# AKGWSB/EzRT

Measured on AMD Instinct MI355X. Metric: Mrays/s at fixed spp (Bunny ~70k tris, 4 bounces), higher is better.
Workload: dtype f32

## Files before the change

### ezrt_amd/csrc/hip/ezrt_device.h

```cpp
#pragma once
#include <hip/hip_runtime.h>
#include <stdint.h>

#include "ezrt.h"
#include "ezrt_detmath.h"

#define EZD __device__ __forceinline__

namespace ezd {

constexpr float PI = EZ_PI;
constexpr float INF = EZ_INF;

struct f3 {
  float x, y, z;
};
EZD f3 mk(float x, float y, float z) { return f3{x, y, z}; }
struct Sample3 {
  float x, y, z;
};
EZD f3 operator+(f3 a, f3 b) { return mk(a.x + b.x, a.y + b.y, a.z + b.z); }
EZD f3 operator-(f3 a, f3 b) { return mk(a.x - b.x, a.y - b.y, a.z - b.z); }
EZD f3 operator*(f3 a, f3 b) { return mk(a.x * b.x, a.y * b.y, a.z * b.z); }
EZD f3 operator*(f3 a, float s) { return mk(a.x * s, a.y * s, a.z * s); }
// ... 16 lines not shown
  return 1.0f / x;
}
EZD f3 normalize(f3 a) {
  float inv = ez_rcp(__builtin_sqrtf(dot(a, a)));
  return a * inv;
}
EZD f3 mix3(f3 a, f3 b, float t) { return mk(ez_mix(a.x, b.x, t), ez_mix(a.y, b.y, t), ez_mix(a.z, b.z, t)); }
EZD f3 reflect(f3 i, f3 n) {
  float k = 2.0f * dot(n, i);
  return i - n * k;
}
EZD float sqr(float x) { return x * x; }

struct DevScene {
  const float4* tri_geom;
  const float* tri_ref;
  const float4* inner;
  const float4* tri_shade;
  const float4* mat_table;
  uint32_t root_ref;
  int32_t n_tri;
  const float4* hdr;
  const uint32_t* hdr_rgbe;
  const float4* cache;
  const float2* cache_xy;
  const float* cache_pdf;
  int32_t env_w, env_h, env_filter;
  uint32_t sobol_mask;
};

template <int INTEG>
constexpr bool integ_mis() { return INTEG == EZRT_INTEGRATOR_P5_MIS || INTEG == EZRT_INTEGRATOR_P5_MIS_ANISO; }
template <int INTEG>
constexpr bool integ_aniso_is() { return INTEG == EZRT_INTEGRATOR_P5_MIS_ANISO; }

struct FastDiv {
  uint32_t d, m, s;
};
inline FastDiv make_fastdiv(uint32_t d) {
  FastDiv f;
  f.d = d ? d : 1u;
  f.m = 0u;
  f.s = 0u;
  if (f.d > 1u) {
    uint32_t L = 0;
    while ((1ull << L) < f.d) L++;
// ... 1194 lines not shown
    float4 p = img[(size_t)iy * W + ix];
    return mk(p.x, p.y, p.z);
  }
  float x = u * (float)W - 0.5f, y = v * (float)H - 0.5f;
  float x0 = ez_floor(x), y0 = ez_floor(y);
  float fx = x - x0, fy = y - y0;
  int ix0 = (int)x0, iy0 = (int)y0, ix1 = ix0 + 1, iy1 = iy0 + 1;
  if (ix0 < 0) ix0 = 0;
  if (iy0 < 0) iy0 = 0;
  if (ix1 > W - 1) ix1 = W - 1;
  if (iy1 > H - 1) iy1 = H - 1;
  float4 p00 = img[(size_t)iy0 * W + ix0], p10 = img[(size_t)iy0 * W + ix1];
  float4 p01 = img[(size_t)iy1 * W + ix0], p11 = img[(size_t)iy1 * W + ix1];
  f3 top = mix3(mk(p00.x, p00.y, p00.z), mk(p10.x, p10.y, p10.z), fx);
  f3 bot = mix3(mk(p01.x, p01.y, p01.z), mk(p11.x, p11.y, p11.z), fx);
  return mix3(top, bot, fy);
}

EZD f3 rgbe_texel(uint32_t p) {
  const int e = (int)(p >> 24) - 136;
  return mk(__builtin_amdgcn_ldexpf((float)(p & 255u), e), __builtin_amdgcn_ldexpf((float)((p >> 8) & 255u), e),
            __builtin_amdgcn_ldexpf((float)((p >> 16) & 255u), e));
}
EZD f3 tex_fetch_rgbe(const uint32_t* __restrict__ img, int W, int H, int filter, float u, float v) {
  u = sane01(u);
  v = sane01(v);
  if (filter == EZRT_FILTER_NEAREST) {
    int ix = (int)ez_floor(u * (float)W), iy = (int)ez_floor(v * (float)H);
    if (ix > W - 1) ix = W - 1;
    if (iy > H - 1) iy = H - 1;
    return rgbe_texel(img[(size_t)iy * W + ix]);
  }
  float x = u * (float)W - 0.5f, y = v * (float)H - 0.5f;
  float x0 = ez_floor(x), y0 = ez_floor(y);
  float fx = x - x0, fy = y - y0;
  int ix0 = (int)x0, iy0 = (int)y0, ix1 = ix0 + 1, iy1 = iy0 + 1;
  if (ix0 < 0) ix0 = 0;
  if (iy0 < 0) iy0 = 0;
  if (ix1 > W - 1) ix1 = W - 1;
  if (iy1 > H - 1) iy1 = H - 1;
  struct __attribute__((packed, aligned(4))) TexelPair {
    uint32_t a, b;
  };
  uint32_t q00, q10, q01, q11;
  if (W >= 2) {
    int bx = ix0 < W - 2 ? ix0 : W - 2;
    const TexelPair r0 = *reinterpret_cast<const TexelPair*>(img + (size_t)iy0 * W + bx);
    const TexelPair r1 = *reinterpret_cast<const TexelPair*>(img + (size_t)iy1 * W + bx);
    q00 = ix0 == bx ? r0.a : r0.b;
    q10 = ix1 == bx ? r0.a : r0.b;
    q01 = ix0 == bx ? r1.a : r1.b;
    q11 = ix1 == bx ? r1.a : r1.b;
  } else {
    q00 = img[(size_t)iy0 * W + ix0], q10 = img[(size_t)iy0 * W + ix1];
    q01 = img[(size_t)iy1 * W + ix0], q11 = img[(size_t)iy1 * W + ix1];
  }
  f3 top = mix3(rgbe_texel(q00), rgbe_texel(q10), fx);
  f3 bot = mix3(rgbe_texel(q01), rgbe_texel(q11), fx);
  return mix3(top, bot, fy);
}

EZD void bilinear_taps(int W, int H, float u, float v, int& ix0, int& ix1, int& iy0, int& iy1, float& fx, float& fy) {
  float x = u * (float)W - 0.5f, y = v * (float)H - 0.5f;
  float x0 = ez_floor(x), y0 = ez_floor(y);
  fx = x - x0;
  fy = y - y0;
  ix0 = (int)x0, iy0 = (int)y0, ix1 = ix0 + 1, iy1 = iy0 + 1;
  if (ix0 < 0) ix0 = 0;
// ... 26 lines not shown
  const Pair r0 = *reinterpret_cast<const Pair*>(img + (size_t)iy0 * W + bx);
  const Pair r1 = *reinterpret_cast<const Pair*>(img + (size_t)iy1 * W + bx);
  const float2 p00 = ix0 == bx ? r0.a : r0.b, p10 = ix1 == bx ? r0.a : r0.b;
  const float2 p01 = ix0 == bx ? r1.a : r1.b, p11 = ix1 == bx ? r1.a : r1.b;
  cx = ez_mix(ez_mix(p00.x, p10.x, fx), ez_mix(p01.x, p11.x, fx), fy);
  cy = ez_mix(ez_mix(p00.y, p10.y, fx), ez_mix(p01.y, p11.y, fx), fy);
}

EZD void to_spherical(f3 v, float& u, float& w) {
  u = ez_atan2(v.z, v.x);
  w = ez_asin(v.y);
  u = u / (2.0f * PI);
  w = w / PI;
  u = u + 0.5f;
  w = w + 0.5f;
  w = 1.0f - w;
}
template <bool FULLCTR>
EZD f3 hdr_color(const DevScene& sc, f3 L, float env_clamp, Counters& ctr) {
  if (FULLCTR) ctr.envmap++;
  if (!sc.hdr) return mk(0, 0, 0);
  float u, v;
  to_spherical(normalize(L), u, v);
  f3 c = sc.hdr_rgbe ? tex_fetch_rgbe(sc.hdr_rgbe, sc.env_w, sc.env_h, sc.env_filter, u, v)
                     : tex_fetch(sc.hdr, sc.env_w, sc.env_h, sc.env_filter, u, v);
  if (env_clamp > 0.0f) c = mk(ez_min(c.x, env_clamp), ez_min(c.y, env_clamp), ez_min(c.z, env_clamp));
  return c;
}
template <bool FULLCTR>
EZD f3 sample_hdr(const DevScene& sc, float xi1, float xi2, Counters& ctr) {
  if (FULLCTR) ctr.envcache++;
  f3 c;
  if (sc.cache_xy && sc.env_filter == EZRT_FILTER_BILINEAR) {
    c.z = 0.0f;
    tex_fetch_xy(sc.cache_xy, sc.env_w, sc.env_h, xi1, xi2, c.x, c.y);
  } else {
    c = tex_fetch(sc.cache, sc.env_w, sc.env_h, sc.env_filter, xi1, xi2);
  }
  float x = c.x, y = 1.0f - c.y;
  float phi = 2.0f * PI * (x - 0.5f);
  float theta = PI * (y - 0.5f);
  float st, ct, sp, cp;
  ez_sincos(theta, &st, &ct);
  ez_sincos(phi, &sp, &cp);
  return mk(ct * cp, st, ct * sp);
}
template <bool FULLCTR>
// ... 1 lines not shown
  if (FULLCTR) ctr.envcache++;
  float u, v;
  to_spherical(normalize(L), u, v);
  float pdf = (sc.cache_pdf && sc.env_filter == EZRT_FILTER_BILINEAR) ? tex_fetch_pdf(sc.cache_pdf, sc.env_w, sc.env_h, u, v)
                                                                     : tex_fetch(sc.cache, sc.env_w, sc.env_h, sc.env_filter, u, v).z;
  float theta = PI * (0.5f - v);
  float sin_theta = ez_max(ez_sin(theta), 1e-10f);
  int res = sc.env_w;
  float p_convert = (float)(res * res / 2) / (2.0f * PI * PI * sin_theta);
  return pdf * p_convert;
}

template <bool FULLCTR>
EZD void hdr_color_pdf(const DevScene& sc, f3 L, float env_clamp, Counters& ctr, f3& color, float& pdf_light) {
  if (FULLCTR) {
    ctr.envmap++;
    ctr.envcache++;
  }
  float u, v;
  to_spherical(normalize(L), u, v);
  if (!sc.hdr) {
    color = mk(0, 0, 0);
  } else {
    f3 c = sc.hdr_rgbe ? tex_fetch_rgbe(sc.hdr_rgbe, sc.env_w, sc.env_h, sc.env_filter, u, v)
                       : tex_fetch(sc.hdr, sc.env_w, sc.env_h, sc.env_filter, u, v);
    if (env_clamp > 0.0f) c = mk(ez_min(c.x, env_clamp), ez_min(c.y, env_clamp), ez_min(c.z, env_clamp));
    color = c;
  }
  float pdf = (sc.cache_pdf && sc.env_filter == EZRT_FILTER_BILINEAR) ? tex_fetch_pdf(sc.cache_pdf, sc.env_w, sc.env_h, u, v)
                                                                     : tex_fetch(sc.cache, sc.env_w, sc.env_h, sc.env_filter, u, v).z;
  float theta = PI * (0.5f - v);
  float sin_theta = ez_max(ez_sin(theta), 1e-10f);
  int res = sc.env_w;
  float p_convert = (float)(res * res / 2) / (2.0f * PI * PI * sin_theta);
  pdf_light = pdf * p_convert;
}

EZD float schlick(float u) {
  float m = ez_clamp(1.0f - u, 0.0f, 1.0f);
  float m2 = m * m;
  return m2 * m2 * m;
}
EZD float gtr1(float NdotH, float a) {
  if (a >= 1.0f) return 1.0f / PI;
  float a2 = a * a;
  float t = 1.0f + (a2 - 1.0f) * NdotH * NdotH;
  return (a2 - 1.0f) / (PI * ez_log(a2) * t);
// ... 267 lines not shown
```

### ezrt_amd/csrc/hip/ezrt_internal.h

```cpp
#pragma once
#include <hip/hip_runtime.h>

#include <algorithm>
#include <array>
#include <chrono>
#include <cstdarg>
#include <cstdio>
#include <cstdlib>
#include <cstring>
#include <exception>
#include <map>
#include <new>
#include <string>
#include <system_error>
#include <thread>
#include <type_traits>
#include <vector>

#include "ezrt.h"
#include "ezrt_device.h"
#include "ezrt_records.h"
#include "ezrt_streams.h"

using namespace ezd;
// ... 125 lines not shown
  int pool_div = 1;
  int pool_min = 8;
  int pool_max = 128;
  int trace_wps_rel = 7;
  int trace_wps = 6;
  int lds_nodes = 1 << 20;
  int scatter = 1;
  int static_pct = 50;
  int refill_min = 24;
  int lazy_dir = 1;
  int regen_dir = 1;
  int refill_min_rel = 40;
  int rel_boxes = 1;
  int steal = 1;
  int wide4 = 1;
  int debug_stages = 0;
  int debug_oom_above = 0;
  int debug_force_pending = 0;
  int shade_wgs = 0;
  int chunk_log2 = 26;
  int launch_events = 0;
  int env_planes = 1;
  int env_rgbe = 1;
  int min_staged = 16;
  int rel_min_records = 4;
  int gen_primary = 1;
  int gen_whole = 1;
  int anyhit = 1;
  int semi = 1;
  int tie_lca = 1;
  int retree = 1;
  int prune = 2;
  int prune_mis = 2;
  int prune_min_records = 0;
  int stack_cap = 0;
  int debug_stack_cap = 0;
  int bounce_scatter = 1;
  int pipeline_calls = 1;
  int static_pct_pipelined = 0;
  int handover = 1;
  int steal_bound = 1;
  int audit_via_queue = 0;
};
struct TuningName {
  const char* name;
  int Tuning::*field;
  int lo, hi;
};
const TuningName kTuning[] = {{"megakernel", &Tuning::megakernel, 0, 1},
                              {"leaf_threshold", &Tuning::leaf_threshold, 1, 64},
                              {"pool_div", &Tuning::pool_div, 1, 1 << 16},
                              {"pool_max", &Tuning::pool_max, 8, 4096},
                              {"pool_min", &Tuning::pool_min, 8, 4096},
                              {"trace_wps", &Tuning::trace_wps, 1, 8},
                              {"trace_wps_rel", &Tuning::trace_wps_rel, 0, 8},
                              {"lds_nodes", &Tuning::lds_nodes, 0, 1 << 24},
                              {"steal", &Tuning::steal, 0, 1},
                              {"rel_boxes", &Tuning::rel_boxes, 0, 1},
                              {"refill_min", &Tuning::refill_min, 1, 64},
                              {"refill_min_rel", &Tuning::refill_min_rel, 0, 64},
                              {"lazy_dir", &Tuning::lazy_dir, 0, 1},
                              {"regen_dir", &Tuning::regen_dir, 0, 1},
                              {"static_pct", &Tuning::static_pct, 0, 95},
                              {"scatter", &Tuning::scatter, 0, 8},
                              {"wide4", &Tuning::wide4, 0, 1},
                              {"debug_stages", &Tuning::debug_stages, 0, 2},
                              {"env_rgbe", &Tuning::env_rgbe, 0, 1},
                              {"env_planes", &Tuning::env_planes, 0, 1},
                              {"launch_events", &Tuning::launch_events, 0, 1},
                              {"shade_wgs", &Tuning::shade_wgs, 0, 4096},
                              {"chunk_log2", &Tuning::chunk_log2, 12, 28},
                              {"debug_force_pending", &Tuning::debug_force_pending, 0, 1 << 20},
                              {"debug_oom_above", &Tuning::debug_oom_above, 0, 1 << 30},
                              {"gen_primary", &Tuning::gen_primary, 0, 1},
                              {"gen_whole", &Tuning::gen_whole, 0, 1},
                              {"rel_min_records", &Tuning::rel_min_records, 0, 4096},
                              {"min_staged", &Tuning::min_staged, 0, 4096},
                              {"anyhit", &Tuning::anyhit, 0, 1},
                              {"semi", &Tuning::semi, 0, 2},
                              {"tie_lca", &Tuning::tie_lca, 0, 1},
                              {"retree", &Tuning::retree, 0, 1},
                              {"prune", &Tuning::prune, 0, 2},
                              {"prune_mis", &Tuning::prune_mis, 0, 2},
                              {"prune_min_records", &Tuning::prune_min_records, 0, 1 << 24},
                              {"stack_cap", &Tuning::stack_cap, 0, 64},
                              {"debug_stack_cap", &Tuning::debug_stack_cap, 0, 8},
                              {"bounce_scatter", &Tuning::bounce_scatter, 0, 1},
                              {"pipeline_calls", &Tuning::pipeline_calls, 0, 2},
                              {"static_pct_pipelined", &Tuning::static_pct_pipelined, 0, 95},
                              {"handover", &Tuning::handover, 0, 1},
                              {"steal_bound", &Tuning::steal_bound, 0, 1},
// ... 84 lines not shown
  DevBuf<int32_t> tri_leaf;
  DevBuf<int2> ref_up;
  DevBuf<float4> inner4;
  int n_inner4 = 0;
  int stack_need4 = 1;
  int stack_need_cp = 1;
  DevBuf<int32_t> cp_uncovered;
  int n_cp_uncovered = 0;
  bool retreed = false;
  bool prunable = false;
  double prune_G = 0.0;
  double prune_Z = 0.0;
  double prune_M = 0.0;
  float prune_a = 0.0f;
  double prune_A_med = 0.0;
  int64_t prune_bad = 0;
  int64_t prune_flagged = 0;
  uint32_t root4 = 0;
  DevBuf<float4> hdr, cache;
  DevBuf<float2> cache_xy;
  DevBuf<float> cache_pdf;
  DevBuf<uint32_t> hdr_rgbe;
  bool has_rgbe = false;
  uint32_t root_ref = 0;
  int env_w = 0, env_h = 0, env_filter = 0;
  bool has_cache = false;
  uint32_t sobol_mask = 7u;
  int instr = 0;
  int depth = 0;
  int64_t stats[6] = {0, 0, 0, 0, 0, 0};
  DevBuf<unsigned long long> counters;
  DevBuf<int2> blocks;
  std::vector<int2> blocks_host;
  EzrtRenderParams blocks_for;
  bool blocks_valid = false;
  DevBuf<float4> accum_tmp;
  Pipe pipe[ezh::SHARED_STREAMS];
  QueryScratch query;
  std::vector<ezi::HostNode> topo_nodes;
  std::vector<int> topo_inner_id;
  std::vector<ezi::HostNode> topo_tree4;
  std::vector<std::array<int, 4>> topo_rec_slots;
  RefitState* refit = nullptr;
  int num_cus = 0;
  uint32_t chunk_seq = 0;
  bool chunk_pipelined = false;
  int n_inner = 0;
  Tuning tune = tuning_from_env();
  hipEvent_t ev_begin = nullptr, ev_end = nullptr;
  hipEvent_t ev_trace[MAX_TRACE_EVENTS][2] = {};
  int n_trace_events = 0, n_trace_launches = 0, n_trace_events_created = 0;
  bool events_ready = false;
  bool timed = false;

  DevScene dev() const {
    DevScene d;
    d.tri_geom = tri_geom.p;
    d.tri_ref = tri_ref.p;
    d.tri_shade = tri_shade.p;
    d.mat_table = mat_table.p;
    d.inner = inner.p;
    d.root_ref = root_ref;
    d.n_tri = n_tri;
    d.hdr = hdr.p;
    d.hdr_rgbe = (has_rgbe && tune.env_rgbe) ? hdr_rgbe.p : nullptr;
    d.cache = has_cache ? cache.p : nullptr;
    d.cache_xy = (has_cache && tune.env_planes && env_w >= 2) ? cache_xy.p : nullptr;
    d.cache_pdf = (has_cache && tune.env_planes && env_w >= 2) ? cache_pdf.p : nullptr;
    d.env_w = env_w;
    d.env_h = env_h;
    d.env_filter = env_filter;
    d.sobol_mask = sobol_mask;
    return d;
  }
};

inline int prune_mode(const EzrtScene* s) {
  if (!s->prunable || s->n_inner4 < s->tune.prune_min_records) return 0;
  return s->tune.prune;
}

namespace ezi {
__attribute__((visibility("hidden"))) void release_chunk_scratch(Pipe& pp);
__attribute__((visibility("hidden"))) bool device_buffer_of(const void* p, size_t bytes, int dev);

inline size_t stack_lds_bytes(const EzrtScene* s) {
  int entries = s->depth > 1 ? s->depth : 1;
  return (size_t)entries * BLOCK * sizeof(int);
// ... 60 lines not shown
```

### ezrt_amd/csrc/hip/ezrt_kernels.h

```cpp
#pragma once
#include "ezrt_device.h"
#include "ezrt_records.h"
#include "ezrt_path_device.h"

namespace ezd {

struct TraceArgs {
  DevScene sc;
  EzrtRenderParams p;
  const int2* blocks;
  int32_t n_blocks;
  uint32_t frame_first;
  Sample3* samples;
  unsigned long long* counters;
  int32_t* log_tri;
  float* log_t;
  float* log_colour;
  int32_t stack_entries;
};

EZD bool pixel_owned(const EzrtRenderParams& p, int x, int y) {
  if (x < p.x0 || x >= p.x1 || y < p.y0 || y >= p.y1) return false;
  if (p.shard_count <= 1) return true;
  int tw = p.tile_w > 0 ? p.tile_w : 32, th = p.tile_h > 0 ? p.tile_h : 32;
// ... 28 lines not shown
  const uint32_t r2 = p - fastdiv(p, n_sub_div) * n_sub;
  return ((fk * n_sub + r2) << sh) | (qslot & ((1u << sh) - 1u));
}

EZD float4 primary_dir(const EzrtRenderParams& p, const int2* blocks, const FastDiv& div_blocks, const FastDiv& div_sub, uint32_t scatter,
                       uint32_t scatter_shift, uint32_t frame_first, uint32_t qslot) {
  int x, y;
  uint32_t frame;
  slot_to_pixel(blocks, div_blocks, queue_to_sample(qslot, div_sub, scatter, scatter_shift), frame_first, x, y, frame);
  if (!pixel_owned(p, x, y)) return make_float4(0, 0, 0, 0.0f);
  uint32_t seed;
  const f3 dir = camera_dir(p, (uint32_t)x, (uint32_t)y, frame, seed);
  return make_float4(dir.x, dir.y, dir.z, 1.0f);
}

struct GenWhole {
  float rot[12];
  float sw, sh;
  FastDiv div_sub, div_bw;
  uint32_t sh_sub, sh_bw;
  uint32_t scatter, scatter_shift, frame_first;
};
template <bool POW2>
EZD void slot_to_pixel_whole(const GenWhole& g, uint32_t qslot, int& x, int& y, uint32_t& frame) {
  const uint32_t sh = g.scatter_shift;
  const uint32_t q = qslot >> sh;
  uint32_t fk, r2;
  if (POW2) {
    fk = q >> g.sh_sub;
    const uint32_t mask = (1u << g.sh_sub) - 1u;
    r2 = ((q & mask) * g.scatter) & mask;
  } else {
    const uint32_t n_sub = g.div_sub.d;
    fk = fastdiv(q, g.div_sub);
    const uint32_t p = (q - fk * n_sub) * g.scatter;
    r2 = p - fastdiv(p, g.div_sub) * n_sub;
  }
  const uint32_t s = (r2 << sh) | (qslot & ((1u << sh) - 1u));
  const uint32_t blk = s >> 8, tid = s & 255u;
  uint32_t bx, by;
  if (POW2) {
    by = blk >> g.sh_bw;
    bx = blk & ((1u << g.sh_bw) - 1u);
  } else {
    by = fastdiv(blk, g.div_bw);
    bx = blk - by * g.div_bw.d;
  }
  const uint32_t wave = tid >> 6, lane = tid & 63u;
  x = (int)(bx * 16u + (wave & 1u) * 8u + (lane & 7u));
  y = (int)(by * 16u + (wave >> 1) * 8u + (lane >> 3));
  frame = g.frame_first + fk;
}
template <bool POW2>
EZD float4 primary_dir_whole(const GenWhole& g, uint32_t qslot, uint32_t& seed) {
  int x, y;
  uint32_t frame;
  slot_to_pixel_whole<POW2>(g, qslot, x, y, frame);
  const f3 dir = camera_dir_scaled<POW2>(g.sw, g.sh, g.rot, (uint32_t)x, (uint32_t)y, frame, seed);
  return make_float4(dir.x, dir.y, dir.z, 1.0f);
}
template <bool POW2>
EZD float4 primary_dir_whole(const GenWhole& g, uint32_t qslot) {
  uint32_t seed;
  return primary_dir_whole<POW2>(g, qslot, seed);
}

template <int INTEG, bool FULLCTR, bool PATHLOG>
__global__ __launch_bounds__(BLOCK) void trace_kernel(TraceArgs a) {
  extern __shared__ __attribute__((aligned(16))) int lds_stack[];
  const int tid = threadIdx.x;
  const int blk = blockIdx.x % a.n_blocks;
  const int fk = blockIdx.x / a.n_blocks;
  const uint32_t frame = a.frame_first + (uint32_t)fk;
  const int wave = tid >> 6, lane = tid & 63;
  const int2 org = a.blocks[blk];
  const int x = org.x + (wave & 1) * 8 + (lane & 7);
  const int y = org.y + (wave >> 1) * 8 + (lane >> 3);
  int* stack = lds_stack + tid;
  const DevScene& sc = a.sc;
  const EzrtRenderParams& p = a.p;
// ... 350 lines not shown
```

### ezrt_amd/csrc/hip/ezrt_scene_build.hip

```cpp
#include "ezrt_internal.h"

namespace {

template <class F>
void parallel_for(int n, int grain, F f) {
  unsigned hw = std::thread::hardware_concurrency();
  if (const char* e = getenv("EZRT_HOST_THREADS")) hw = (unsigned)std::max(1, atoi(e));
  int nt = (int)std::min<unsigned>(hw ? hw : 1u, 16u);
  nt = std::min(nt, std::max(1, n / std::max(1, grain)));
  if (nt <= 1) {
    f(0, n, 0);
    return;
  }
  std::vector<std::thread> th;
  std::vector<std::exception_ptr> err((size_t)nt);
  th.reserve((size_t)nt);
  for (int k = 0; k < nt; k++) {
    const int lo = (int)((long long)n * k / nt), hi = (int)((long long)n * (k + 1) / nt);
    auto body = [=, &f, &err] {
      try {
        f(lo, hi, k);
      } catch (...) {
        err[(size_t)k] = std::current_exception();
      }
// ... 759 lines not shown
  s->topo_rec_slots = std::move(rec_slot_nodes);
  lap("device allocation + upload");
  s->stats[0] = n_tri;
  s->stats[1] = n_nodes;
  s->stats[2] = maxd;
  s->stats[3] = leaves;
  s->stats[4] = maxleaf;
  s->stats[5] = (int64_t)(geom.size() * sizeof(float4) + (size_t)n_tri * 144 + inner.size() * sizeof(float4) +
                          inner4.size() * sizeof(float4) + shade.size() * sizeof(float4) + mats.size() * sizeof(float4));
  *out = s;
  return 0;
}

static int ezrt_scene_set_env_body(EzrtScene* s, const float* hdr, const float* cache, int w, int h, int filter) {
  if (!s || !hdr || w <= 0 || h <= 0) return fail(EZRT_ERR_INVALID, "bad env arguments");
  if (filter != EZRT_FILTER_NEAREST && filter != EZRT_FILTER_BILINEAR) return fail(EZRT_ERR_INVALID, "bad filter");
  if ((int64_t)w * w / 2 >= ((int64_t)1 << 31)) return fail(EZRT_ERR_UNSUPPORTED, "hdrResolution^2/2 overflows int");
  size_t n = (size_t)w * h;
  std::vector<float4> tmp(n);
  for (size_t i = 0; i < n; i++) tmp[i] = make_float4(hdr[i * 3], hdr[i * 3 + 1], hdr[i * 3 + 2], 0.0f);
  HIP_TRY(s->hdr.ensure(n));
  HIP_TRY(hipMemcpy(s->hdr.p, tmp.data(), n * sizeof(float4), hipMemcpyHostToDevice));
  s->has_rgbe = false;
  {
    std::vector<uint32_t> packed(n);
    bool ok = true;
    for (size_t i = 0; i < n && ok; i++) {
      const float c[3] = {hdr[i * 3], hdr[i * 3 + 1], hdr[i * 3 + 2]};
      uint32_t bits[3];
      memcpy(bits, c, sizeof bits);
      if ((bits[0] | bits[1] | bits[2]) == 0u) {
        packed[i] = 0u;
        continue;
      }
      float mx = c[0] > c[1] ? c[0] : c[1];
      mx = mx > c[2] ? mx : c[2];
      if (!(mx > 0.0f) || !(c[0] >= 0.0f) || !(c[1] >= 0.0f) || !(c[2] >= 0.0f) || mx > 3.0e38f) {
        ok = false;
        break;
      }
      int k = 0;
      (void)frexpf(mx, &k);
      const int E = k + 128;
      if (E < 0 || E > 255) {
        ok = false;
        break;
      }
      uint32_t m[3];
      for (int j = 0; j < 3 && ok; j++) {
        if (bits[j] == 0x80000000u) ok = false;
        const float q = ldexpf(c[j], 8 - k);
        const uint32_t mi = (uint32_t)q;
        if (!(q >= 0.0f && q < 256.0f) || (float)mi != q || ldexpf((float)mi, E - 136) != c[j]) ok = false;
        m[j] = mi;
      }
      if (ok) packed[i] = m[0] | (m[1] << 8) | (m[2] << 16) | ((uint32_t)E << 24);
    }
    if (ok) {
      HIP_TRY(s->hdr_rgbe.ensure(n));
      HIP_TRY(hipMemcpy(s->hdr_rgbe.p, packed.data(), n * sizeof(uint32_t), hipMemcpyHostToDevice));
      s->has_rgbe = true;
    }
  }
  s->has_cache = false;
  if (cache) {
    for (size_t i = 0; i < n; i++) tmp[i] = make_float4(cache[i * 3], cache[i * 3 + 1], cache[i * 3 + 2], 0.0f);
    HIP_TRY(s->cache.ensure(n));
    HIP_TRY(hipMemcpy(s->cache.p, tmp.data(), n * sizeof(float4), hipMemcpyHostToDevice));
    {
      std::vector<float2> xy(n);
      std::vector<float> pdf(n);
      for (size_t i = 0; i < n; i++) {
        xy[i] = make_float2(cache[i * 3], cache[i * 3 + 1]);
        pdf[i] = cache[i * 3 + 2];
      }
      HIP_TRY(s->cache_xy.ensure(n));
      HIP_TRY(s->cache_pdf.ensure(n));
      HIP_TRY(hipMemcpy(s->cache_xy.p, xy.data(), n * sizeof(float2), hipMemcpyHostToDevice));
      HIP_TRY(hipMemcpy(s->cache_pdf.p, pdf.data(), n * sizeof(float), hipMemcpyHostToDevice));
    }
    s->has_cache = true;
  }
  s->env_w = w;
  s->env_h = h;
// ... 9 lines not shown
```

### ezrt_amd/csrc/hip/ezrt_traceq4.h

```cpp
#pragma once
#include "ezrt_records.h"
#include "ezrt_traceq.h"

namespace ezd {

struct TraceQ4Args {
  TraceQArgs q;
  const float4* inner4;
  const float4* inner4_rel;
  uint32_t root4;
  int32_t lds_nodes4;
  float prune_a, prune_cs;
  const int32_t* tri_leaf;
  const int2* ref_up;
  struct GenGeneral {
    EzrtRenderParams p;
    const int2* blocks;
    FastDiv div_blocks, div_sub;
    uint32_t scatter, scatter_shift, frame_first;
  };
  union {
    GenGeneral gen;
    GenWhole gen_whole;
  };
// ... 176 lines not shown
      best_tri = tri;
      tie_tri = -1;
      if (PRUNE) prune_t = hw_min(prune_t, (t + pdelta) * PRUNE_REL);
    } else if (!OCC && t == best_t && tri != best_tri) {
      if (A.tri_leaf && tie_tri < 0) tie_tri = tri;
      else if (tri != tie_tri) tie = true;
    }
  };

  const unsigned long long t_start = (LOG && a.wave_log) ? wall_clock64() : 0ull;
  unsigned long long t_exhausted = 0ull;
  uint32_t wave_iters = 0, dbg_inner_lanes = 0, dbg_inner_steps = 0, dbg_leaf_lanes = 0, dbg_leaf_rounds = 0, dbg_busy_lanes = 0,
           dbg_refills = 0, dbg_steals = 0, dbg_max_sp = 0;
  for (;;) {
    if (LOG) wave_iters++;
    const bool want = ref >= REF_DONE;
    const unsigned long long wantm = ballot(want);
    if (wantm && ((uint32_t)__popcll(wantm) >= a.refill_min || !ballot(ref < REF_DONE))) {
      if (LOG && a.wave_log) dbg_refills++;
      if (ref == REF_DONE) publish();
      if (ref == REF_NONE && nx_slot != REF_NONE) {
        const uint32_t adopted = nx_slot;
        nx_slot = REF_NONE;
        if (nx_d.w != 0.0f) {
          n_counted += a.count_rays;
          slot = adopted;
          S = REL ? mk(a.origin[0], a.origin[1], a.origin[2]) : mk(nx_o.x, nx_o.y, nx_o.z);
          d = mk(nx_d.x, nx_d.y, nx_d.z);
          inv = mk(ez_rcp(d.x), ez_rcp(d.y), ez_rcp(d.z));
          best_t = OCC ? nx_o.w : INF;
          best_tri = -1;
          sp = 0;
          sb = 0;
          semi = SEMI && ray_is_semi(S, d, inv);
          anyhit = a.anyhit_even != 0u && (adopted & 1u) == 0u;
          tie = !(ray_is_tame(S, inv) || semi) || (a.force_pending && adopted % a.force_pending == 0u);
          tie_tri = -1;
          ref = tie ? REF_DONE : A.root4;
          best_tri = tie ? HIT_PENDING : -1;
          if (PRUNE) set_delta();
        }
      }
      const bool need = nx_slot == REF_NONE && !exhausted;
      const unsigned long long m = ballot(need);
      if (m) {
        const uint32_t cnt = (uint32_t)__popcll(m);
// ... 16 lines not shown
          const uint32_t left = pool_end - pool_next;
          uint32_t take_n = cnt - left;
          if (take_n > pool_size) take_n = pool_size;
          idx = (r < left) ? (pool_next + r) : (base + (r - left));
          served = r < left + take_n;
          pool_next = base + take_n;
          pool_end = base + pool_size;
          if (base >= n_rays) exhausted = true;
        } else {
          idx = pool_next + r;
          served = true;
          pool_next += cnt;
          if (pool_next >= n_rays && pool_end >= n_rays) exhausted = true;
        }
        uint32_t rs = idx;
        if (gscat) {
          const uint32_t g = idx >> GSH;
          rs = (((g & 255u) * (n_rays >> (8u + GSH)) + (g >> 8)) << GSH) | (idx & ((1u << GSH) - 1u));
        }
        if (need && served && idx < n_rays && rs < n_real) {
          if (a.slot_map) rs = a.slot_map[idx];
          nx_slot = rs;
          if (!REL) nx_o = a.const_origin == 1u ? make_float4(a.origin[0], a.origin[1], a.origin[2], 0.0f) : a.rq.o[rs >> (a.const_origin >> 1)];
          if (GEN) {
            if (WHOLE) nx_d = primary_dir_whole<WHOLE >= 2>(A.gen_whole, rs);
            else nx_d = primary_dir(A.gen.p, A.gen.blocks, A.gen.div_blocks, A.gen.div_sub, A.gen.scatter, A.gen.scatter_shift, A.gen.frame_first, rs);
            if (WHOLE != 3) a.rq.d[rs] = nx_d;
          } else {
            nx_d = a.rq.d[rs];
          }
        }
      }
    }
    if (!ballot((ref & nx_slot) != REF_NONE)) {
      if (!exhausted) continue;
      break;
    }
    if (LOG && a.wave_log && exhausted && !t_exhausted) t_exhausted = wall_clock64();

    if (a.steal && exhausted) {
      if (A.handover) {
        const bool idle0 = (ref & nx_slot) == REF_NONE;
        const bool host = nx_slot != REF_NONE && ref < REF_DONE;
        const unsigned long long im0 = ballot(idle0), hm = ballot(host);
        if (im0 && hm) {
          const int ni0 = (int)__popcll(im0), nh = (int)__popcll(hm);
          const int n0 = ni0 < nh ? ni0 : nh;
          const int ir0 = (int)lane_rank(im0), hr = (int)lane_rank(hm);
          const bool giver = host && hr < n0, taker = idle0 && ir0 < n0;
          if (giver) wsrc[hr] = lane;
          __builtin_amdgcn_wave_barrier();
          const int src = taker ? wsrc[ir0] : lane;
          const uint32_t hs = (uint32_t)__shfl((int)nx_slot, src, 64);
          const float hdx = __shfl(nx_d.x, src, 64), hdy = __shfl(nx_d.y, src, 64), hdz = __shfl(nx_d.z, src, 64), hdw = __shfl(nx_d.w, src, 64);
          float hox = 0.0f, hoy = 0.0f, hoz = 0.0f, how = 0.0f;
          if (!REL) hox = __shfl(nx_o.x, src, 64), hoy = __shfl(nx_o.y, src, 64), hoz = __shfl(nx_o.z, src, 64);
          if (OCC) how = __shfl(nx_o.w, src, 64);
          __builtin_amdgcn_wave_barrier();
          if (giver) nx_slot = REF_NONE;
          if (taker) {
            nx_slot = hs;
            nx_d = make_float4(hdx, hdy, hdz, hdw);
            if (!REL) nx_o = make_float4(hox, hoy, hoz, how);
          }
        }
      }
      const bool idle = (ref & nx_slot) == REF_NONE;
      const unsigned long long im = ballot(idle);
      if (im) {
        const bool rich = sp > sb;
        const unsigned long long vm = ballot(rich);
        const int ni = (int)__popcll(im), nv = (int)__popcll(vm);
        const int n = ni < nv ? ni : nv;
        const int ir = (int)lane_rank(im), vr = (int)lane_rank(vm);
        if (n) {
          if (LOG && a.wave_log) dbg_steals++;
          const bool victim = rich && vr < n, thief = idle && ir < n;
          int give = 0;
          if (victim) {
            wsrc[vr] = lane;
            give = stack[(sb & ring_mask) * BLOCK];
            sb++;
            if (!shared) atomicExch(&hits64[slot], ~0ull);
            shared = true;
          }
// ... 239 lines not shown
```

### ezrt_amd/csrc/hip/ezrt_wavefront.h

```cpp
#pragma once
#include "ezrt_kernels.h"
#include "ezrt_traceq.h"
#include "ezrt_traceq4.h"

namespace ezd {

constexpr uint32_t FLAG_SHADOW_SHOT = 1u;
constexpr uint32_t FLAG_TERMINATE = 2u;
constexpr uint32_t FLAG_PDF_DEAD = 4u;
struct PathState {
  float4* s0;
  float4* s1;
  float4* s2;
  float4* s3;
  float4* s4;
};
template <int INTEG>
constexpr bool compact_state() { return INTEG == EZRT_INTEGRATOR_P5_SOBOL; }
template <int INTEG, int STAGE>
constexpr bool mis_stage1_state() { return integ_mis<INTEG>() && STAGE == 1; }
struct WfArgs {
  DevScene sc;
  EzrtRenderParams p;
  const int2* blocks;
// ... 91 lines not shown
    uint32_t t = 0;
    for (int w = 0; w < NW; w++) {
      uint32_t c = lds[w];
      lds[w] = t;
      t += c;
    }
    lds[NW] = t;
  }
  __syncthreads();
  total = lds[NW];
  return lds[wave] + lane_rank(m);
}

struct ShadeOut {
  bool emit;
  uint32_t sslot, seed, flags, tri0;
  f3 history, Lo, Le0, f_r, shadowC, rayL, shadowL, P;
  float cosine, pdf;
};

struct ShadeIn {
  float4 rd4, ro4, s0, s1, s2, s3, s4;
  int2 h, sh;
};
template <int INTEG, int PASS, int STAGE, bool REGEN = false>
EZD void shade_load(const WfArgs& a, const uint32_t i, const bool live, ShadeIn& in, const uint4* entry = nullptr) {
  constexpr bool MIS = integ_mis<INTEG>();
  constexpr bool B0 = (STAGE == 0);
  constexpr bool COMPACT = compact_state<INTEG>();
  constexpr bool MIS1 = mis_stage1_state<INTEG, STAGE>();
  const EzrtRenderParams& p = a.p;
  const int b = a.bounce;
  const uint32_t ii = live ? i : 0u;
  const uint32_t rslot = (b == 0 || !MIS) ? ii : (2u * ii + 1u);
  const bool from_entry = PASS == 2 && entry && (int32_t)entry->y != HIT_PENDING && (!MIS || (int32_t)entry->w != HIT_PENDING);
  int2 h = from_entry ? make_int2((int32_t)entry->y, (int32_t)entry->z) : a.hits[rslot];
  float4 rd4;
  static_assert(!REGEN || (B0 && PASS != 0), "the regenerating instances are the primary stage's two passes");
  if constexpr (REGEN) {
    rd4 = make_float4(0.0f, 0.0f, 0.0f, 1.0f);
  } else if (B0 && PASS == 1 && a.all_owned) {
    asm volatile("" : "+v"(h.x), "+v"(h.y));
    rd4 = make_float4(0.0f, 0.0f, 0.0f, 1.0f);
    if (h.x < 0) rd4 = a.rq_in.d[rslot];
  } else {
    rd4 = a.rq_in.d[rslot];
// ... 2 lines not shown
  float4 ro4 = make_float4(p.eye[0], p.eye[1], p.eye[2], 0.0f);
  float4 s0 = make_float4(0, 0, 0, 0), s1 = s0, s2 = s0, s3 = s0, s4 = s0;
  int2 sh = make_int2(-1, 0);
  if (!B0) {
    if (PASS != 1) ro4 = a.rq_in.o[ii];
    if (!COMPACT && !MIS1) s3 = a.st_in.s3[ii];
    s0 = a.st_in.s0[ii];
    if (COMPACT && STAGE == 1) {
      if (!lean) {
        const float2 q = reinterpret_cast<const float2*>(a.st_in.s1)[ii];
        s1 = make_float4(q.x, q.y, 0.0f, 0.0f);
      }
    } else {
      s1 = a.st_in.s1[ii];
    }
    if ((!COMPACT || STAGE >= 2) && !MIS1) s2 = a.st_in.s2[ii];
    if (MIS) {
      s4 = a.st_in.s4[ii];
      sh = from_entry ? make_int2((int32_t)entry->w, 0) : a.hits[2u * ii];
    }
  }
  if constexpr (REGEN && PASS == 2) {
    uint32_t seed;
    rd4 = primary_dir_whole<true>(a.gen_whole, rslot, seed);
    s3.w = __uint_as_float(seed);
  }
#define EZ_PIN4(v) asm volatile("" : "+v"(v.x), "+v"(v.y), "+v"(v.z), "+v"(v.w))
  if constexpr (!REGEN) EZ_PIN4(rd4);
  asm volatile("" : "+v"(h.x), "+v"(h.y));
  if (!B0) {
    if (PASS != 1) EZ_PIN4(ro4);
    EZ_PIN4(s0);
    if (!lean) EZ_PIN4(s1);
    if ((!COMPACT || STAGE >= 2) && !MIS1) EZ_PIN4(s2);
    if (!COMPACT && !MIS1) EZ_PIN4(s3);
    if (MIS) {
      EZ_PIN4(s4);
      asm volatile("" : "+v"(sh.x), "+v"(sh.y));
    }
  }
#undef EZ_PIN4
  if (lean) {
    const uint32_t w = __float_as_uint(rd4.w);
    uint32_t t0 = 0xffffffffu;
    if (w & LEAN_EMITS) t0 = __float_as_uint(PASS == 1 ? reinterpret_cast<const float*>(a.rq_in.o + ii)[3] : ro4.w);
    s1 = make_float4(__uint_as_float(w & LEAN_SLOT_MASK), __uint_as_float(t0), 0.0f, 0.0f);
  }
// ... 12 lines not shown
EZD bool shade_body(const WfArgs& a, const uint32_t i, bool live, const ShadeIn& in, Counters& ctr, uint32_t& n_samples,
                    ShadeOut& o) {
  constexpr bool P5TRI = (INTEG >= 50);
  constexpr bool MIS = integ_mis<INTEG>();
  const DevScene& sc = a.sc;
  const EzrtRenderParams& p = a.p;
  const int b = a.bounce;
  constexpr bool B0 = (STAGE == 0);
  constexpr bool COMPACT = compact_state<INTEG>();
  uint32_t sslot = 0, seed = 0, flags = 0, tri0 = 0;
  f3 history = mk(1, 1, 1), Lo = mk(0, 0, 0), Le0 = mk(0, 0, 0), f_r = mk(0, 0, 0), shadowC = mk(0, 0, 0);
  float cosine = 0.0f, pdf = 1.0f;
  f3 rayL = mk(0, 0, 0), shadowL = mk(0, 0, 0);
  Hit hit;
  hit.P = mk(0, 0, 0);
  o.emit = false;
  const float4 rd4 = in.rd4, ro4 = in.ro4, s0 = in.s0, s1 = in.s1, s2 = in.s2, s3 = in.s3, s4 = in.s4;
  const int2 h = in.h, sh = in.sh;
  bool done = false;
  if (!live) return false;
  f3 colour = mk(0, 0, 0);
  f3 rd = mk(rd4.x, rd4.y, rd4.z);
  if (B0) {
    sslot = queue_to_sample(i, a.div_sub, a.scatter, a.scatter_shift);
    if (rd4.w == 0.0f) {
      live = false;
    } else {
      if (PASS != 2) n_samples = n_samples + 1;
      if (PASS == 1 && h.x == HIT_PENDING) return true;
      if (h.x < 0) {
        if constexpr (REGEN && PASS == 1) {
          const float4 g = primary_dir_whole<true>(a.gen_whole, i);
          rd = mk(g.x, g.y, g.z);
        }
        colour = hdr_color<FULLCTR>(sc, rd, p.env_clamp, ctr);
        done = true;
      } else {
        if (PASS == 1) return true;
        shade_point<P5TRI>(sc, h.x, __int_as_float(h.y), mk(ro4.x, ro4.y, ro4.z), rd, hit);
        Le0 = hit.m.emissive;
        tri0 = (__float_as_uint(Le0.x) | __float_as_uint(Le0.y) | __float_as_uint(Le0.z)) ? (uint32_t)h.x : 0xffffffffu;
        if constexpr (REGEN) {
          seed = __float_as_uint(s3.w);
        } else if (INTEG != EZRT_INTEGRATOR_P5_SOBOL) {
          int x0, y0;
          uint32_t f0;
          slot_to_pixel(a.blocks, a.div_blocks, sslot, a.frame_first, x0, y0, f0);
// ... 72 lines not shown
          Lo = Lo + (((history * w) * sky) * f_r) * cosine / pdf;
        } else {
          Lo = Lo + ((history * sky) * f_r) * cosine / pdf;
        }
        done = true;
      } else {
        if (PASS == 1) return true;
        shade_point<P5TRI>(sc, h.x, __int_as_float(h.y), mk(ro4.x, ro4.y, ro4.z), rd, hit);
        Lo = Lo + ((history * hit.m.emissive) * f_r) * cosine / pdf;
        history = history * (f_r * cosine / pdf);
      }
    }
    if (done) colour = Le0 + Lo;
  }
  if (live && !done && b >= p.max_bounce) {
    colour = Le0 + Lo;
    done = true;
  }
  if (live && done) a.samples[sslot] = Sample3{colour.x, colour.y, colour.z};

  if (live && !done) {
    int x, y;
    uint32_t frame;
    slot_to_pixel(a.blocks, a.div_blocks, sslot, a.frame_first, x, y, frame);
    const f3 V = -hit.viewDir, N = hit.N;
    constexpr bool ANISO_IS = integ_aniso_is<INTEG>();
    f3 X = mk(0, 0, 0), Y = mk(0, 0, 0);
    if (ANISO_IS) get_tangent(N, X, Y);
    flags = 0;
    bool shoot = true;
    if (MIS) {
      float h1 = rnd(seed);
      float h2 = rnd(seed);
      f3 Lh = sample_hdr<FULLCTR>(sc, h1, h2, ctr);
      if (dot(N, Lh) > 0.0f) {
        flags |= FLAG_SHADOW_SHOT;
        shadowL = Lh;
        Counters dummy = {0, 0, 0, 0, 0, 0, 0};
        f3 color;
        float pdf_light;
        hdr_color_pdf<false>(sc, Lh, p.env_clamp, dummy, color, pdf_light);
        f3 fr;
        float pdf_brdf;
        brdf_evaluate_pdf<ANISO_IS>(V, N, Lh, X, Y, hit.m, fr, pdf_brdf);
        float w = mis_mix_weight(pdf_light, pdf_brdf);
        shadowC = (((history * w) * color) * fr) * dot(N, Lh) / pdf_light;
      }
// ... 396 lines not shown
```

Before: 15680.

## Add row-paired RGBE env texels and reuse regenerated primary pixel coords

Builds a host-side env map layout that stores each texel together with the texel in the row below, so a bilinear fetch becomes one 16-byte load instead of two 8-byte loads. In the shading kernel it reuses the pixel, frame and sample slot computed during primary-ray regeneration instead of recomputing them with division-based index math. In the traversal queue it defers primary direction generation until a slot is adopted, and stops shuffling directions between lanes in GEN mode. The env pair layout doubles env map memory, and moving direction generation changes when and where it runs.

Result: faster. 15970, median of 6 (+1.8%).

```diff
diff --git a/ezrt_amd/csrc/hip/ezrt_device.h b/ezrt_amd/csrc/hip/ezrt_device.h
--- a/ezrt_amd/csrc/hip/ezrt_device.h
+++ b/ezrt_amd/csrc/hip/ezrt_device.h
@@ -62,6 +62,7 @@
   int32_t n_tri;
   const float4* hdr;
   const uint32_t* hdr_rgbe;
+  const uint2* hdr_pairs;
   const float4* cache;
   const float2* cache_xy;
   const float* cache_pdf;
@@ -1302,7 +1303,7 @@
   return mk(__builtin_amdgcn_ldexpf((float)(p & 255u), e), __builtin_amdgcn_ldexpf((float)((p >> 8) & 255u), e),
             __builtin_amdgcn_ldexpf((float)((p >> 16) & 255u), e));
 }
-EZD f3 tex_fetch_rgbe(const uint32_t* __restrict__ img, int W, int H, int filter, float u, float v) {
+EZD f3 tex_fetch_rgbe(const uint32_t* __restrict__ img, const uint2* __restrict__ pairs, int W, int H, int filter, float u, float v) {
   u = sane01(u);
   v = sane01(v);
   if (filter == EZRT_FILTER_NEAREST) {
@@ -1323,7 +1324,17 @@
     uint32_t a, b;
   };
   uint32_t q00, q10, q01, q11;
-  if (W >= 2) {
+  if (pairs) {
+    struct __attribute__((packed, aligned(8))) PairPair {
+      uint32_t a_top, a_bot, b_top, b_bot;
+    };
+    const int bx = ix0 < W - 2 ? ix0 : W - 2;
+    const PairPair r = *reinterpret_cast<const PairPair*>(pairs + (size_t)((int)y0 + 1) * W + bx);
+    q00 = ix0 == bx ? r.a_top : r.b_top;
+    q10 = ix1 == bx ? r.a_top : r.b_top;
+    q01 = ix0 == bx ? r.a_bot : r.b_bot;
+    q11 = ix1 == bx ? r.a_bot : r.b_bot;
+  } else if (W >= 2) {
     int bx = ix0 < W - 2 ? ix0 : W - 2;
     const TexelPair r0 = *reinterpret_cast<const TexelPair*>(img + (size_t)iy0 * W + bx);
     const TexelPair r1 = *reinterpret_cast<const TexelPair*>(img + (size_t)iy1 * W + bx);
@@ -1396,7 +1407,7 @@
   if (!sc.hdr) return mk(0, 0, 0);
   float u, v;
   to_spherical(normalize(L), u, v);
-  f3 c = sc.hdr_rgbe ? tex_fetch_rgbe(sc.hdr_rgbe, sc.env_w, sc.env_h, sc.env_filter, u, v)
+  f3 c = sc.hdr_rgbe ? tex_fetch_rgbe(sc.hdr_rgbe, sc.hdr_pairs, sc.env_w, sc.env_h, sc.env_filter, u, v)
                      : tex_fetch(sc.hdr, sc.env_w, sc.env_h, sc.env_filter, u, v);
   if (env_clamp > 0.0f) c = mk(ez_min(c.x, env_clamp), ez_min(c.y, env_clamp), ez_min(c.z, env_clamp));
   return c;
@@ -1444,7 +1455,7 @@
   if (!sc.hdr) {
     color = mk(0, 0, 0);
   } else {
-    f3 c = sc.hdr_rgbe ? tex_fetch_rgbe(sc.hdr_rgbe, sc.env_w, sc.env_h, sc.env_filter, u, v)
+    f3 c = sc.hdr_rgbe ? tex_fetch_rgbe(sc.hdr_rgbe, sc.hdr_pairs, sc.env_w, sc.env_h, sc.env_filter, u, v)
                        : tex_fetch(sc.hdr, sc.env_w, sc.env_h, sc.env_filter, u, v);
     if (env_clamp > 0.0f) c = mk(ez_min(c.x, env_clamp), ez_min(c.y, env_clamp), ez_min(c.z, env_clamp));
     color = c;
diff --git a/ezrt_amd/csrc/hip/ezrt_internal.h b/ezrt_amd/csrc/hip/ezrt_internal.h
--- a/ezrt_amd/csrc/hip/ezrt_internal.h
+++ b/ezrt_amd/csrc/hip/ezrt_internal.h
@@ -171,6 +171,7 @@
   int launch_events = 0;
   int env_planes = 1;
   int env_rgbe = 1;
+  int env_pairs = 1;
   int min_staged = 16;
   int rel_min_records = 4;
   int gen_primary = 1;
@@ -216,6 +217,7 @@
                               {"debug_stages", &Tuning::debug_stages, 0, 2},
                               {"env_rgbe", &Tuning::env_rgbe, 0, 1},
                               {"env_planes", &Tuning::env_planes, 0, 1},
+                              {"env_pairs", &Tuning::env_pairs, 0, 1},
                               {"launch_events", &Tuning::launch_events, 0, 1},
                               {"shade_wgs", &Tuning::shade_wgs, 0, 4096},
                               {"chunk_log2", &Tuning::chunk_log2, 12, 28},
@@ -346,6 +348,8 @@
   DevBuf<float> cache_pdf;
   DevBuf<uint32_t> hdr_rgbe;
   bool has_rgbe = false;
+  DevBuf<uint2> hdr_pairs;
+  bool has_pairs = false;
   uint32_t root_ref = 0;
   int env_w = 0, env_h = 0, env_filter = 0;
   bool has_cache = false;
@@ -388,6 +392,7 @@
     d.n_tri = n_tri;
     d.hdr = hdr.p;
     d.hdr_rgbe = (has_rgbe && tune.env_rgbe) ? hdr_rgbe.p : nullptr;
+    d.hdr_pairs = (has_pairs && tune.env_rgbe && tune.env_pairs) ? hdr_pairs.p : nullptr;
     d.cache = has_cache ? cache.p : nullptr;
     d.cache_xy = (has_cache && tune.env_planes && env_w >= 2) ? cache_xy.p : nullptr;
     d.cache_pdf = (has_cache && tune.env_planes && env_w >= 2) ? cache_pdf.p : nullptr;
diff --git a/ezrt_amd/csrc/hip/ezrt_kernels.h b/ezrt_amd/csrc/hip/ezrt_kernels.h
--- a/ezrt_amd/csrc/hip/ezrt_kernels.h
+++ b/ezrt_amd/csrc/hip/ezrt_kernels.h
@@ -74,7 +74,7 @@
   uint32_t scatter, scatter_shift, frame_first;
 };
 template <bool POW2>
-EZD void slot_to_pixel_whole(const GenWhole& g, uint32_t qslot, int& x, int& y, uint32_t& frame) {
+EZD void slot_to_pixel_whole(const GenWhole& g, uint32_t qslot, int& x, int& y, uint32_t& frame, uint32_t& sslot) {
   const uint32_t sh = g.scatter_shift;
   const uint32_t q = qslot >> sh;
   uint32_t fk, r2;
@@ -102,12 +102,24 @@
   x = (int)(bx * 16u + (wave & 1u) * 8u + (lane & 7u));
   y = (int)(by * 16u + (wave >> 1) * 8u + (lane >> 3));
   frame = g.frame_first + fk;
+  sslot = ((POW2 ? fk << g.sh_sub : fk * g.div_sub.d) << sh) + s;
+}
+template <bool POW2>
+EZD void slot_to_pixel_whole(const GenWhole& g, uint32_t qslot, int& x, int& y, uint32_t& frame) {
+  uint32_t sslot;
+  slot_to_pixel_whole<POW2>(g, qslot, x, y, frame, sslot);
 }
 template <bool POW2>
 EZD float4 primary_dir_whole(const GenWhole& g, uint32_t qslot, uint32_t& seed) {
   int x, y;
   uint32_t frame;
   slot_to_pixel_whole<POW2>(g, qslot, x, y, frame);
+  const f3 dir = camera_dir_scaled<POW2>(g.sw, g.sh, g.rot, (uint32_t)x, (uint32_t)y, frame, seed);
+  return make_float4(dir.x, dir.y, dir.z, 1.0f);
+}
+template <bool POW2>
+EZD float4 primary_dir_whole(const GenWhole& g, uint32_t qslot, uint32_t& seed, int& x, int& y, uint32_t& frame, uint32_t& sslot) {
+  slot_to_pixel_whole<POW2>(g, qslot, x, y, frame, sslot);
   const f3 dir = camera_dir_scaled<POW2>(g.sw, g.sh, g.rot, (uint32_t)x, (uint32_t)y, frame, seed);
   return make_float4(dir.x, dir.y, dir.z, 1.0f);
 }
diff --git a/ezrt_amd/csrc/hip/ezrt_scene_build.hip b/ezrt_amd/csrc/hip/ezrt_scene_build.hip
--- a/ezrt_amd/csrc/hip/ezrt_scene_build.hip
+++ b/ezrt_amd/csrc/hip/ezrt_scene_build.hip
@@ -805,6 +805,7 @@
   HIP_TRY(s->hdr.ensure(n));
   HIP_TRY(hipMemcpy(s->hdr.p, tmp.data(), n * sizeof(float4), hipMemcpyHostToDevice));
   s->has_rgbe = false;
+  s->has_pairs = false;
   {
     std::vector<uint32_t> packed(n);
     bool ok = true;
@@ -843,6 +844,17 @@
       HIP_TRY(s->hdr_rgbe.ensure(n));
       HIP_TRY(hipMemcpy(s->hdr_rgbe.p, packed.data(), n * sizeof(uint32_t), hipMemcpyHostToDevice));
       s->has_rgbe = true;
+      if (w >= 2) {
+        std::vector<uint2> pairs((size_t)(h + 1) * w);
+        for (int j = 0; j <= h; j++) {
+          const uint32_t* top = packed.data() + (size_t)(j > 0 ? j - 1 : 0) * w;
+          const uint32_t* bot = packed.data() + (size_t)(j < h ? j : h - 1) * w;
+          for (int x = 0; x < w; x++) pairs[(size_t)j * w + x] = make_uint2(top[x], bot[x]);
+        }
+        HIP_TRY(s->hdr_pairs.ensure(pairs.size()));
+        HIP_TRY(hipMemcpy(s->hdr_pairs.p, pairs.data(), pairs.size() * sizeof(uint2), hipMemcpyHostToDevice));
+        s->has_pairs = true;
+      }
     }
   }
   s->has_cache = false;
diff --git a/ezrt_amd/csrc/hip/ezrt_traceq4.h b/ezrt_amd/csrc/hip/ezrt_traceq4.h
--- a/ezrt_amd/csrc/hip/ezrt_traceq4.h
+++ b/ezrt_amd/csrc/hip/ezrt_traceq4.h
@@ -222,6 +222,11 @@
       if (ref == REF_NONE && nx_slot != REF_NONE) {
         const uint32_t adopted = nx_slot;
         nx_slot = REF_NONE;
+        if constexpr (GEN) {
+          if (WHOLE) nx_d = primary_dir_whole<WHOLE >= 2>(A.gen_whole, adopted);
+          else nx_d = primary_dir(A.gen.p, A.gen.blocks, A.gen.div_blocks, A.gen.div_sub, A.gen.scatter, A.gen.scatter_shift, A.gen.frame_first, adopted);
+          if (WHOLE != 3) a.rq.d[adopted] = nx_d;
+        }
         if (nx_d.w != 0.0f) {
           n_counted += a.count_rays;
           slot = adopted;
@@ -284,13 +289,7 @@
           if (a.slot_map) rs = a.slot_map[idx];
           nx_slot = rs;
           if (!REL) nx_o = a.const_origin == 1u ? make_float4(a.origin[0], a.origin[1], a.origin[2], 0.0f) : a.rq.o[rs >> (a.const_origin >> 1)];
-          if (GEN) {
-            if (WHOLE) nx_d = primary_dir_whole<WHOLE >= 2>(A.gen_whole, rs);
-            else nx_d = primary_dir(A.gen.p, A.gen.blocks, A.gen.div_blocks, A.gen.div_sub, A.gen.scatter, A.gen.scatter_shift, A.gen.frame_first, rs);
-            if (WHOLE != 3) a.rq.d[rs] = nx_d;
-          } else {
-            nx_d = a.rq.d[rs];
-          }
+          if constexpr (!GEN) nx_d = a.rq.d[rs];
         }
       }
     }
@@ -314,7 +313,8 @@
           __builtin_amdgcn_wave_barrier();
           const int src = taker ? wsrc[ir0] : lane;
           const uint32_t hs = (uint32_t)__shfl((int)nx_slot, src, 64);
-          const float hdx = __shfl(nx_d.x, src, 64), hdy = __shfl(nx_d.y, src, 64), hdz = __shfl(nx_d.z, src, 64), hdw = __shfl(nx_d.w, src, 64);
+          float hdx = 0.0f, hdy = 0.0f, hdz = 0.0f, hdw = 0.0f;
+          if constexpr (!GEN) hdx = __shfl(nx_d.x, src, 64), hdy = __shfl(nx_d.y, src, 64), hdz = __shfl(nx_d.z, src, 64), hdw = __shfl(nx_d.w, src, 64);
           float hox = 0.0f, hoy = 0.0f, hoz = 0.0f, how = 0.0f;
           if (!REL) hox = __shfl(nx_o.x, src, 64), hoy = __shfl(nx_o.y, src, 64), hoz = __shfl(nx_o.z, src, 64);
           if (OCC) how = __shfl(nx_o.w, src, 64);
@@ -322,7 +322,7 @@
           if (giver) nx_slot = REF_NONE;
           if (taker) {
             nx_slot = hs;
-            nx_d = make_float4(hdx, hdy, hdz, hdw);
+            if constexpr (!GEN) nx_d = make_float4(hdx, hdy, hdz, hdw);
             if (!REL) nx_o = make_float4(hox, hoy, hoz, how);
           }
         }
diff --git a/ezrt_amd/csrc/hip/ezrt_wavefront.h b/ezrt_amd/csrc/hip/ezrt_wavefront.h
--- a/ezrt_amd/csrc/hip/ezrt_wavefront.h
+++ b/ezrt_amd/csrc/hip/ezrt_wavefront.h
@@ -137,6 +137,8 @@
 struct ShadeIn {
   float4 rd4, ro4, s0, s1, s2, s3, s4;
   int2 h, sh;
+  int gen_x, gen_y;
+  uint32_t gen_frame, gen_sslot;
 };
 template <int INTEG, int PASS, int STAGE, bool REGEN = false>
 EZD void shade_load(const WfArgs& a, const uint32_t i, const bool live, ShadeIn& in, const uint4* entry = nullptr) {
@@ -185,7 +187,7 @@
   }
   if constexpr (REGEN && PASS == 2) {
     uint32_t seed;
-    rd4 = primary_dir_whole<true>(a.gen_whole, rslot, seed);
+    rd4 = primary_dir_whole<true>(a.gen_whole, rslot, seed, in.gen_x, in.gen_y, in.gen_frame, in.gen_sslot);
     s3.w = __uint_as_float(seed);
   }
 #define EZ_PIN4(v) asm volatile("" : "+v"(v.x), "+v"(v.y), "+v"(v.z), "+v"(v.w))
@@ -244,7 +246,17 @@
   f3 colour = mk(0, 0, 0);
   f3 rd = mk(rd4.x, rd4.y, rd4.z);
   if (B0) {
-    sslot = queue_to_sample(i, a.div_sub, a.scatter, a.scatter_shift);
+    if constexpr (REGEN) {
+      if (PASS == 2) {
+        sslot = in.gen_sslot;
+      } else {
+        int gx, gy;
+        uint32_t gf;
+        slot_to_pixel_whole<true>(a.gen_whole, i, gx, gy, gf, sslot);
+      }
+    } else {
+      sslot = queue_to_sample(i, a.div_sub, a.scatter, a.scatter_shift);
+    }
     if (rd4.w == 0.0f) {
       live = false;
     } else {
@@ -363,7 +375,8 @@
   if (live && !done) {
     int x, y;
     uint32_t frame;
-    slot_to_pixel(a.blocks, a.div_blocks, sslot, a.frame_first, x, y, frame);
+    if constexpr (REGEN && PASS == 2) x = in.gen_x, y = in.gen_y, frame = in.gen_frame;
+    else slot_to_pixel(a.blocks, a.div_blocks, sslot, a.frame_first, x, y, frame);
     const f3 V = -hit.viewDir, N = hit.N;
     constexpr bool ANISO_IS = integ_aniso_is<INTEG>();
     f3 X = mk(0, 0, 0), Y = mk(0, 0, 0);
```
